# chaitjo/efficient-gnns

Measured on NVIDIA H100. Metric: edges aggregated/s (fwd+bwd), 3-layer GCN student + logit-KD, ARXIV-shape, higher is better.
Workload: dtype f32

## Files before the change

efficient-gnns_b200/csrc/gemm_wgrad_tf32x3.cu:

```cuda
#include "common.cuh"
#include "tc_common.cuh"

namespace b200gnn {
namespace wgrad {
using namespace tc;

constexpr int BKN = 32;
constexpr int TM = 128, TN = 128;
constexpr int THREADS = 384;
constexpr int STAGES = 5;
constexpr int X_BOX = 8;
constexpr int RAW_BYTES = BKN * (TM + TN) * 4;
constexpr int OP_BYTES = 128 * BKN * 4;
constexpr int T_BYTES = 2 * OP_BYTES;
constexpr int SS_BYTES = TM / 2 * 16;
constexpr int SMEM_BYTES = STAGES * RAW_BYTES + 2 * T_BYTES + 256 + SS_BYTES + 1024;
constexpr int MAX_RANGES = 132;
constexpr int64_t MAX_PARTIAL_FLOATS = (int64_t)MAX_RANGES * 256 * 256;
constexpr int MAX_KIN = 2048, MAX_NOUT = 512;
static_assert(SMEM_BYTES <= 232448, "shared memory");

struct Params {
  float* partial;
  int32_t Nn, Kin, Kpad, Nout, Npad, num_kb;
  int32_t n_tn, n_ranges;
  const float* act_scale;
  const float* act_shift;
  const uint32_t* act_bits;
  int32_t act_words;
  float inv_keep;
  const float* act_slope;
  int32_t act_ld;
};

template <bool ACT, bool PRELU = false>
__global__ void __launch_bounds__(THREADS, 1)
wgrad_tf32x3_kernel(const __grid_constant__ CUtensorMap tmX, const __grid_constant__ CUtensorMap tmG, const Params p) {
  extern __shared__ uint8_t smem_raw[];
  uint8_t* smem = reinterpret_cast<uint8_t*>((reinterpret_cast<uintptr_t>(smem_raw) + 1023) & ~(uintptr_t)1023);
  uint8_t* tbuf = smem + STAGES * RAW_BYTES;
  uint64_t* full = reinterpret_cast<uint64_t*>(tbuf + 2 * T_BYTES);
  uint64_t* empty = full + STAGES;
  float4* act_ss = reinterpret_cast<float4*>(tbuf + 2 * T_BYTES + 256);

  const int tiles = (p.Kpad / TM) * p.n_tn;
  const int tile = (int)blockIdx.x % tiles, range = (int)blockIdx.x / tiles;
  const int mt = tile / p.n_tn, nt = tile % p.n_tn;
  const int kb0 = (int)((int64_t)p.num_kb * range / p.n_ranges);
  const int kb1 = (int)((int64_t)p.num_kb * (range + 1) / p.n_ranges);

  const int warp = threadIdx.x >> 5, lane = threadIdx.x & 31;
  if (threadIdx.x == 0) {
    for (int s = 0; s < STAGES; ++s) { mbar_init(&full[s], 1); mbar_init(&empty[s], 256); }
    asm volatile("fence.mbarrier_init.release.cluster;" ::: "memory");
  }
  __syncthreads();

  if (warp < 4) {
    regs_dec<40>();
    if (threadIdx.x == 0) {
      int s = 0; uint32_t ph = 0;
      for (int kb = kb0; kb < kb1; ++kb) {
        mbar_wait(&empty[s], ph ^ 1);
        uint8_t* st = smem + s * RAW_BYTES;
        mbar_expect_tx(&full[s], RAW_BYTES);
        for (int j = 0; j < TM / X_BOX; ++j)
          tma_load_2d(&tmX, &full[s], st + j * BKN * X_BOX * 4, mt * TM + j * X_BOX, kb * BKN);
        tma_load_2d(&tmG, &full[s], st + BKN * TM * 4, nt * TN, kb * BKN);
        if (++s == STAGES) { s = 0; ph ^= 1; }
      }
    }
    return;
  }
  regs_inc<232>();

  const int cw = (warp >> 2) - 1;
  const int ct = threadIdx.x - 128;
  const uint32_t xfrag = (8 * cw + 2 * (warp & 3)) * (BKN * X_BOX * 4) + (lane & 3) * (X_BOX * 4) + (lane >> 2) * 4;
  const int pair = cw * 32 + (warp & 3) * 8 + (lane >> 2);
  const int c0 = mt * TM + cw * 64 + (warp & 3) * 16 + (lane >> 2);
  uint32_t wnext = 0u;
  const int bits_ld = PRELU ? p.act_ld : p.act_words;
  auto act_word = [&](int kb) {
    const int node = kb * BKN + lane;
    return node < p.Nn && (c0 >> 5) < p.act_words ? __ldg(p.act_bits + (size_t)node * bits_ld + (c0 >> 5)) : 0u;
  };
  const float slope = PRELU ? __ldg(p.act_slope) : 0.f;
  if (PRELU && kb0 < kb1) wnext = act_word(kb0);
  if (ACT) {
    if (ct < TM / 2) {
      const int c = mt * TM + (ct >> 3) * 16 + (ct & 7);
      float4 v = make_float4(0.f, 0.f, 0.f, 0.f);
      if (c < p.Kin) { v.x = __ldg(p.act_scale + c); v.y = __ldg(p.act_shift + c); }
      if (c + 8 < p.Kin) { v.z = __ldg(p.act_scale + c + 8); v.w = __ldg(p.act_shift + c + 8); }
      act_ss[ct] = v;
    }
    if (kb0 < kb1) wnext = act_word(kb0);
    named_sync(1, 256);
  }
  float acc[64], sum[64];
#pragma unroll
  for (int i = 0; i < 64; ++i) sum[i] = acc[i] = 0.f;
  uint32_t xh0[BKN / 8][4], xl0[BKN / 8][4], xh1[BKN / 8][4], xl1[BKN / 8][4];
  int s = 0; uint32_t ph = 0;
  auto block = [&](int i, uint32_t (&h)[BKN / 8][4], uint32_t (&l)[BKN / 8][4]) {
    uint32_t wcur = 0u;
    if (ACT || PRELU) {
      wcur = wnext;
      if (kb0 + i + 1 < kb1) wnext = act_word(kb0 + i + 1);
    }
    mbar_wait(&full[s], ph);
    float4 ss = make_float4(0.f, 0.f, 0.f, 0.f);
    int l4 = lane & 3;
    if (ACT) {
      ss = act_ss[pair];
      asm volatile("" : "+r"(l4));
    }
    if (PRELU) asm volatile("" : "+r"(l4));
    const uint32_t sraw = smem_u32(smem + s * RAW_BYTES);
    const float* rg = reinterpret_cast<const float*>(smem + s * RAW_BYTES + BKN * TM * 4);
    uint8_t* T = tbuf + (i & 1) * T_BYTES;
#pragma unroll
    for (int u = 0; u < 4; ++u) {
      const int idx = u * 256 + ct;
      const int r = idx & 127, c = idx >> 7;
      const float* src = rg + (4 * c) * 128 + r;
      const uint4 v = make_uint4(__float_as_uint(src[0]), __float_as_uint(src[128]), __float_as_uint(src[256]),
                                 __float_as_uint(src[384]));
      uint4 hv, lv;
      split4(v, hv, lv);
      *reinterpret_cast<uint4*>(T + swz128(r, c)) = hv;
      *reinterpret_cast<uint4*>(T + OP_BYTES + swz128(r, c)) = lv;
    }
#pragma unroll
    for (int k = 0; k < BKN / 8; ++k)
#pragma unroll
      for (int j = 0; j < 4; ++j) {
        uint32_t v = lds32(sraw + xfrag + (j & 1) * (BKN * X_BOX * 4) + (8 * k + 4 * (j >> 1)) * (X_BOX * 4));
        if (ACT) {
          const uint32_t w = __shfl_sync(0xffffffffu, wcur, 8 * k + l4 + 4 * (j >> 1));
          const float y = fmaxf(fmaf(__uint_as_float(v), (j & 1) ? ss.z : ss.x, (j & 1) ? ss.w : ss.y), 0.f) * p.inv_keep;
          v = (w >> ((c0 & 31) + 8 * (j & 1))) & 1u ? __float_as_uint(y) : 0u;
        }
        if (PRELU) {
          const uint32_t w = __shfl_sync(0xffffffffu, wcur, 8 * k + l4 + 4 * (j >> 1));
          const float z = __uint_as_float(v);
          const float y = (z > 0.f ? z : slope * z) * p.inv_keep;
          v = (w >> ((c0 & 31) + 8 * (j & 1))) & 1u ? __float_as_uint(y) : 0u;
        }
        split1(v, h[k][j], l[k][j]);
      }
    asm volatile("fence.proxy.async.shared::cta;" ::: "memory");
    mbar_arrive(&empty[s]);
    if (i > 0) {
      wgmma_wait<0>();
      acc_fence(acc);
#pragma unroll
      for (int j = 0; j < 64; ++j) sum[j] += acc[j];
    }
    named_sync(1, 256);
    reg_fence(h); reg_fence(l);
    wgmma_fence();
    const uint32_t sa = smem_u32(T);
#pragma unroll
    for (int k = 0; k < BKN / 8; ++k) {
      const uint32_t koff = k * 32;
      wgmma_tf32_n128_rs(acc, l[k], make_desc_k128(sa + koff), k != 0);
      wgmma_tf32_n128_rs(acc, h[k], make_desc_k128(sa + OP_BYTES + koff), 1);
    }
#pragma unroll
    for (int k = 0; k < BKN / 8; ++k) wgmma_tf32_n128_rs(acc, h[k], make_desc_k128(sa + k * 32), 1);
    wgmma_commit();
    if (++s == STAGES) { s = 0; ph ^= 1; }
  };
  for (int i = 0; i < kb1 - kb0; i += 2) {
    block(i, xh0, xl0);
    if (i + 1 < kb1 - kb0) block(i + 1, xh1, xl1);
  }
  if (kb1 > kb0) {
    wgmma_wait<0>();
    acc_fence(acc);
#pragma unroll
    for (int j = 0; j < 64; ++j) sum[j] += acc[j];
  }
  float* out = p.partial + (size_t)range * p.Kpad * p.Npad;
  const int row0 = mt * TM + cw * 64 + (warp & 3) * 16 + (lane >> 2);
#pragma unroll
  for (int j = 0; j < 16; ++j) {
    const int col = nt * TN + 8 * j + 2 * (lane & 3);
    if (col < p.Npad) {
      *reinterpret_cast<float2*>(out + (size_t)row0 * p.Npad + col) = make_float2(sum[4 * j], sum[4 * j + 1]);
      *reinterpret_cast<float2*>(out + (size_t)(row0 + 8) * p.Npad + col) = make_float2(sum[4 * j + 2], sum[4 * j + 3]);
    }
  }
}

constexpr int RED_VECS = 32, RED_GROUPS = 8;
__global__ void __launch_bounds__(RED_VECS * RED_GROUPS) wgrad_reduce_kernel(const float4* __restrict__ partial, int n_part,
                                                                             int Kin, int Kpad, int Nout, int Npad,
                                                                             float* __restrict__ out) {
  __shared__ float4 sh[RED_GROUPS][RED_VECS];
  const int64_t n_vec = (int64_t)Kpad * Npad / 4;
  const int v = threadIdx.x % RED_VECS, g = threadIdx.x / RED_VECS;
  const int64_t i = (int64_t)blockIdx.x * RED_VECS + v;
  float4 acc = make_float4(0.f, 0.f, 0.f, 0.f);
  if (i < n_vec)
    for (int c = g; c < n_part; c += RED_GROUPS) {
      const float4 x = __ldcs(partial + (size_t)c * n_vec + i);
      acc.x += x.x; acc.y += x.y; acc.z += x.z; acc.w += x.w;
    }
  sh[g][v] = acc;
  __syncthreads();
  if (g != 0 || i >= n_vec) return;
  const int row = (int)(i / (Npad / 4)), c4 = (int)(i % (Npad / 4)) * 4;
  if (c4 >= Nout || row >= Kin) return;
#pragma unroll
  for (int j = 1; j < RED_GROUPS; ++j) {
    const float4 x = sh[j][v];
    acc.x += x.x; acc.y += x.y; acc.z += x.z; acc.w += x.w;
  }
  *reinterpret_cast<float4*>(out + (size_t)row * Nout + c4) = acc;
}

static bool make_map_rows(CUtensorMap* m, const float* base, int64_t rows, int64_t width, int64_t ld, int box_cols) {
  EncodeTiledFn fn = encode_fn();
  if (!fn) return false;
  cuuint64_t dims[2] = {(cuuint64_t)width, (cuuint64_t)rows};
  cuuint64_t strides[1] = {(cuuint64_t)ld * 4};
  cuuint32_t box[2] = {(cuuint32_t)box_cols, (cuuint32_t)BKN};
  cuuint32_t estr[2] = {1, 1};
  return fn(m, CU_TENSOR_MAP_DATA_TYPE_FLOAT32, 2, const_cast<float*>(base), dims, strides, box, estr,
            CU_TENSOR_MAP_INTERLEAVE_NONE, CU_TENSOR_MAP_SWIZZLE_NONE, CU_TENSOR_MAP_L2_PROMOTION_L2_256B,
            CU_TENSOR_MAP_FLOAT_OOB_FILL_NONE) == CUDA_SUCCESS;
}

static int64_t pad_k(int64_t Kin) { return (Kin + TM - 1) / TM * TM; }
static int64_t pad_n(int64_t Nout) { return (Nout + 31) / 32 * 32; }
static int range_cap(int64_t Kin, int64_t Nout) {
  const int64_t c = MAX_PARTIAL_FLOATS / (pad_k(Kin) * pad_n(Nout));
  return (int)(c > MAX_RANGES ? MAX_RANGES : (c < 1 ? 1 : c));
}

}
}

using namespace b200gnn;

extern "C" int64_t b200gnn_wgrad_workspace_floats(int64_t Kin, int64_t Nout) {
  if (Kin <= 0 || Nout <= 0) return B200GNN_ERR_BAD_ARG;
  if (Kin > wgrad::MAX_KIN || Nout > wgrad::MAX_NOUT) return B200GNN_ERR_UNSUPPORTED;
  return wgrad::range_cap(Kin, Nout) * wgrad::pad_k(Kin) * wgrad::pad_n(Nout);
}

template <bool ACT, bool PRELU = false>
static int wgrad_launch(const float* X, int64_t ldx, const float* G, int64_t ldg, float* dW, int64_t Nn, int64_t Kin, int64_t Nout,
                        float* workspace, const wgrad::Params& act, void* stream) {
  if (!X || !G || !dW || !workspace || Nn <= 0 || Kin <= 0 || Nout <= 0 || ldx < Kin || ldg < Nout || Nn >= INT32_MAX)
    return B200GNN_ERR_BAD_ARG;
  if (Kin % 4 || Kin > wgrad::MAX_KIN || Nout % 4 || Nout > wgrad::MAX_NOUT || ldx % 4 || ldg % 4 || !aligned_to(X, 16) || !aligned_to(G, 16) ||
      !aligned_to(dW, 16) || !aligned_to(workspace, 16))
    return B200GNN_ERR_UNSUPPORTED;
  CUtensorMap tX, tG;
  if (!wgrad::make_map_rows(&tX, X, Nn, Kin, ldx, wgrad::X_BOX) || !wgrad::make_map_rows(&tG, G, Nn, Nout, ldg, wgrad::TN))
    return B200GNN_ERR_UNSUPPORTED;
  int dev = 0, sms = 132;
  cudaGetDevice(&dev);
  static bool attr_set[64] = {};
  if (dev >= 0 && dev < 64 && !attr_set[dev]) {
    cudaError_t e = cudaFuncSetAttribute(wgrad::wgrad_tf32x3_kernel<ACT, PRELU>, cudaFuncAttributeMaxDynamicSharedMemorySize,
                                         wgrad::SMEM_BYTES);
    if (e != cudaSuccess) { set_cuda_error(e); return B200GNN_ERR_CUDA; }
    attr_set[dev] = true;
  }
  cudaDeviceGetAttribute(&sms, cudaDevAttrMultiProcessorCount, dev);
  cudaStream_t st = (cudaStream_t)stream;
  wgrad::Params p = act;
  p.partial = workspace; p.Nn = (int32_t)Nn; p.Kin = (int32_t)Kin; p.Nout = (int32_t)Nout;
  p.Kpad = (int32_t)wgrad::pad_k(Kin);
  p.Npad = (int32_t)wgrad::pad_n(Nout);
  p.num_kb = (int32_t)((Nn + wgrad::BKN - 1) / wgrad::BKN);
  p.n_tn = (p.Npad + wgrad::TN - 1) / wgrad::TN;
  const int tiles = (int)(p.Kpad / wgrad::TM) * p.n_tn;
  int ranges = sms / tiles;
  const int cap = wgrad::range_cap(Kin, Nout);
  if (ranges > cap) ranges = cap;
  if (ranges > p.num_kb) ranges = p.num_kb;
  if (ranges < 1) ranges = 1;
  p.n_ranges = ranges;
  int rc;
  wgrad::wgrad_tf32x3_kernel<ACT, PRELU><<<tiles * ranges, wgrad::THREADS, wgrad::SMEM_BYTES, st>>>(tX, tG, p);
  if ((rc = check_launch())) return rc;
  const int64_t n_vec = (int64_t)p.Kpad * p.Npad / 4;
  wgrad::wgrad_reduce_kernel<<<(int)((n_vec + wgrad::RED_VECS - 1) / wgrad::RED_VECS), wgrad::RED_VECS * wgrad::RED_GROUPS, 0, st>>>(
      reinterpret_cast<const float4*>(workspace), ranges, (int)Kin, p.Kpad, (int)Nout, p.Npad, dW);
  return check_launch();
}

extern "C" int b200gnn_gemm_wgrad_tf32x3_f32(const float* X, int64_t ldx, const float* G, int64_t ldg, float* dW,
                                             int64_t Nn, int64_t Kin, int64_t Nout, float* workspace, void* stream) {
  return wgrad_launch<false>(X, ldx, G, ldg, dW, Nn, Kin, Nout, workspace, wgrad::Params{}, stream);
}

extern "C" int b200gnn_gemm_wgrad_tf32x3_act_f32(const float* Y, int64_t ldx, const float* G, int64_t ldg, float* dW,
                                                 int64_t Nn, int64_t Kin, int64_t Nout, const float* scale, const float* shift,
                                                 const uint32_t* bits, float p_drop, float* workspace, void* stream) {
  if (!scale || !shift || !bits || p_drop < 0.f || p_drop >= 1.f) return B200GNN_ERR_BAD_ARG;
  wgrad::Params act{};
  act.act_scale = scale; act.act_shift = shift; act.act_bits = bits; act.act_words = (int32_t)((Kin + 31) / 32);
  act.inv_keep = p_drop > 0.f ? 1.f / (1.f - p_drop) : 1.f;
  return wgrad_launch<true>(Y, ldx, G, ldg, dW, Nn, Kin, Nout, workspace, act, stream);
}

extern "C" int b200gnn_gemm_wgrad_tf32x3_prelu_f32(const float* Z, int64_t ldz, const float* G, int64_t ldg, float* dW,
                                                   int64_t Nn, int64_t Kin, int64_t Nout, const float* slope,
                                                   const uint32_t* bits, int64_t ldbits, float p_drop, float* workspace,
                                                   void* stream) {
  if (!slope || !bits || ldbits < (Kin + 31) / 32 || ldbits >= INT32_MAX || p_drop < 0.f || p_drop >= 1.f)
    return B200GNN_ERR_BAD_ARG;
  wgrad::Params act{};
  act.act_slope = slope; act.act_bits = bits; act.act_words = (int32_t)((Kin + 31) / 32); act.act_ld = (int32_t)ldbits;
  act.inv_keep = p_drop > 0.f ? 1.f / (1.f - p_drop) : 1.f;
  return wgrad_launch<false, true>(Z, ldz, G, ldg, dW, Nn, Kin, Nout, workspace, act, stream);
}
```

Baseline: 3.973 billion.

## Add narrow N=48 wgrad tile and offload half of transpose to producer warps

Templates the weight-gradient kernel on output tile width and dispatches a 48-wide tile (deeper pipeline, n48 wgmma) when Nout is small, as for the 40-class ArXiv output layer, instead of padding to 128. The G transpose/split work is also divided between the idle producer-side warps (96 threads) and the consumer warpgroups, coordinated by new tfull/tempty mbarriers that replace the named barrier. This cuts wasted MMA work on narrow outputs and overlaps the transpose with compute, at the cost of a more complex barrier protocol and some ablation macros left in the code.

```diff
diff --git a/efficient-gnns_b200/csrc/gemm_wgrad_tf32x3.cu b/efficient-gnns_b200/csrc/gemm_wgrad_tf32x3.cu
--- a/efficient-gnns_b200/csrc/gemm_wgrad_tf32x3.cu
+++ b/efficient-gnns_b200/csrc/gemm_wgrad_tf32x3.cu
@@ -1,24 +1,55 @@
 #include "common.cuh"
 #include "tc_common.cuh"
+
+#ifndef WGRAD_ABLATE
+#define WGRAD_ABLATE 0
+#endif
 
 namespace b200gnn {
 namespace wgrad {
 using namespace tc;
 
 constexpr int BKN = 32;
-constexpr int TM = 128, TN = 128;
+constexpr int TM = 128;
 constexpr int THREADS = 384;
-constexpr int STAGES = 5;
+constexpr int TRANSPOSERS = 96;
 constexpr int X_BOX = 8;
-constexpr int RAW_BYTES = BKN * (TM + TN) * 4;
-constexpr int OP_BYTES = 128 * BKN * 4;
-constexpr int T_BYTES = 2 * OP_BYTES;
 constexpr int SS_BYTES = TM / 2 * 16;
-constexpr int SMEM_BYTES = STAGES * RAW_BYTES + 2 * T_BYTES + 256 + SS_BYTES + 1024;
+constexpr int BAR_BYTES = 256;
+template <int TN>
+struct Tile {
+  static constexpr int STAGES = TN == 128 ? 5 : 8;
+  static constexpr int RAW_BYTES = BKN * (TM + TN) * 4;
+  static constexpr int OP_BYTES = TN * BKN * 4;
+  static constexpr int T_BYTES = 2 * OP_BYTES;
+  static constexpr int ACC = TN / 2;
+  static constexpr int SMEM_BYTES = STAGES * RAW_BYTES + 2 * T_BYTES + BAR_BYTES + SS_BYTES + 1024;
+  static_assert((STAGES * RAW_BYTES) % 1024 == 0 && OP_BYTES % 1024 == 0, "swizzled T tiles start on 1024-byte atoms");
+  static_assert((2 * STAGES + 4) * 8 <= BAR_BYTES, "barrier block");
+  static_assert(SMEM_BYTES <= 232448, "shared memory");
+};
 constexpr int MAX_RANGES = 132;
 constexpr int64_t MAX_PARTIAL_FLOATS = (int64_t)MAX_RANGES * 256 * 256;
 constexpr int MAX_KIN = 2048, MAX_NOUT = 512;
-static_assert(SMEM_BYTES <= 232448, "shared memory");
+
+__device__ __forceinline__ void mma(float (&d)[64], const uint32_t (&a)[4], uint64_t b, uint32_t s) { wgmma_tf32_n128_rs(d, a, b, s); }
+__device__ __forceinline__ void mma(float (&d)[24], const uint32_t (&a)[4], uint64_t b, uint32_t s) { wgmma_tf32_n48_rs(d, a, b, s); }
+
+template <int TN, int UNROLL>
+__device__ __forceinline__ void transpose_split(const float* rg, uint8_t* T, int idx, int end, int step) {
+  constexpr int OP_BYTES = TN * BKN * 4;
+#pragma unroll UNROLL
+  for (; idx < end; idx += step) {
+    const int r = idx % TN, c = idx / TN;
+    const float* src = rg + (4 * c) * TN + r;
+    const uint4 v = make_uint4(__float_as_uint(src[0]), __float_as_uint(src[TN]), __float_as_uint(src[2 * TN]),
+                               __float_as_uint(src[3 * TN]));
+    uint4 hv, lv;
+    split4(v, hv, lv);
+    *reinterpret_cast<uint4*>(T + swz128(r, c)) = hv;
+    *reinterpret_cast<uint4*>(T + OP_BYTES + swz128(r, c)) = lv;
+  }
+}
 
 struct Params {
   float* partial;
@@ -33,15 +64,19 @@
   int32_t act_ld;
 };
 
-template <bool ACT, bool PRELU = false>
+template <int TN, bool ACT, bool PRELU>
 __global__ void __launch_bounds__(THREADS, 1)
 wgrad_tf32x3_kernel(const __grid_constant__ CUtensorMap tmX, const __grid_constant__ CUtensorMap tmG, const Params p) {
+  using T_ = Tile<TN>;
+  constexpr int STAGES = T_::STAGES, RAW_BYTES = T_::RAW_BYTES, OP_BYTES = T_::OP_BYTES, T_BYTES = T_::T_BYTES;
   extern __shared__ uint8_t smem_raw[];
   uint8_t* smem = reinterpret_cast<uint8_t*>((reinterpret_cast<uintptr_t>(smem_raw) + 1023) & ~(uintptr_t)1023);
   uint8_t* tbuf = smem + STAGES * RAW_BYTES;
   uint64_t* full = reinterpret_cast<uint64_t*>(tbuf + 2 * T_BYTES);
   uint64_t* empty = full + STAGES;
-  float4* act_ss = reinterpret_cast<float4*>(tbuf + 2 * T_BYTES + 256);
+  uint64_t* tfull = empty + STAGES;
+  uint64_t* tempty = tfull + 2;
+  float4* act_ss = reinterpret_cast<float4*>(tbuf + 2 * T_BYTES + BAR_BYTES);
 
   const int tiles = (p.Kpad / TM) * p.n_tn;
   const int tile = (int)blockIdx.x % tiles, range = (int)blockIdx.x / tiles;
@@ -51,7 +86,8 @@
 
   const int warp = threadIdx.x >> 5, lane = threadIdx.x & 31;
   if (threadIdx.x == 0) {
-    for (int s = 0; s < STAGES; ++s) { mbar_init(&full[s], 1); mbar_init(&empty[s], 256); }
+    for (int s = 0; s < STAGES; ++s) { mbar_init(&full[s], 1); mbar_init(&empty[s], 256 + TRANSPOSERS); }
+    for (int t = 0; t < 2; ++t) { mbar_init(&tfull[t], TRANSPOSERS + 8); mbar_init(&tempty[t], 8); }
     asm volatile("fence.mbarrier_init.release.cluster;" ::: "memory");
   }
   __syncthreads();
@@ -67,6 +103,20 @@
         for (int j = 0; j < TM / X_BOX; ++j)
           tma_load_2d(&tmX, &full[s], st + j * BKN * X_BOX * 4, mt * TM + j * X_BOX, kb * BKN);
         tma_load_2d(&tmG, &full[s], st + BKN * TM * 4, nt * TN, kb * BKN);
+        if (++s == STAGES) { s = 0; ph ^= 1; }
+      }
+    } else if (warp > 0) {
+      const int tt = threadIdx.x - 32;
+      int s = 0; uint32_t ph = 0;
+      for (int i = 0; i < kb1 - kb0; ++i) {
+        const float* rg = reinterpret_cast<const float*>(smem + s * RAW_BYTES + BKN * TM * 4);
+        uint8_t* T = tbuf + (i & 1) * T_BYTES;
+        mbar_wait(&tempty[i & 1], ((i >> 1) & 1) ^ 1);
+        mbar_wait(&full[s], ph);
+        transpose_split<TN, 2>(rg, T, TN * BKN / 8 + tt, TN * BKN / 4 * (WGRAD_ABLATE != 2), TRANSPOSERS);
+        asm volatile("fence.proxy.async.shared::cta;" ::: "memory");
+        mbar_arrive(&empty[s]);
+        mbar_arrive(&tfull[i & 1]);
         if (++s == STAGES) { s = 0; ph ^= 1; }
       }
     }
@@ -98,9 +148,10 @@
     if (kb0 < kb1) wnext = act_word(kb0);
     named_sync(1, 256);
   }
-  float acc[64], sum[64];
-#pragma unroll
-  for (int i = 0; i < 64; ++i) sum[i] = acc[i] = 0.f;
+  constexpr int ACC = T_::ACC;
+  float acc[ACC], sum[ACC];
+#pragma unroll
+  for (int i = 0; i < ACC; ++i) sum[i] = acc[i] = 0.f;
   uint32_t xh0[BKN / 8][4], xl0[BKN / 8][4], xh1[BKN / 8][4], xl1[BKN / 8][4];
   int s = 0; uint32_t ph = 0;
   auto block = [&](int i, uint32_t (&h)[BKN / 8][4], uint32_t (&l)[BKN / 8][4]) {
@@ -117,21 +168,13 @@
       asm volatile("" : "+r"(l4));
     }
     if (PRELU) asm volatile("" : "+r"(l4));
+    mbar_wait(&tempty[i & 1], ((i >> 1) & 1) ^ 1);
+    transpose_split<TN, 1>(reinterpret_cast<const float*>(smem + s * RAW_BYTES + BKN * TM * 4), tbuf + (i & 1) * T_BYTES, ct,
+                        TN * BKN / 8 * (WGRAD_ABLATE != 2), 256);
+    asm volatile("fence.proxy.async.shared::cta;" ::: "memory");
+    __syncwarp();
+    if (lane == 0) mbar_arrive(&tfull[i & 1]);
     const uint32_t sraw = smem_u32(smem + s * RAW_BYTES);
-    const float* rg = reinterpret_cast<const float*>(smem + s * RAW_BYTES + BKN * TM * 4);
-    uint8_t* T = tbuf + (i & 1) * T_BYTES;
-#pragma unroll
-    for (int u = 0; u < 4; ++u) {
-      const int idx = u * 256 + ct;
-      const int r = idx & 127, c = idx >> 7;
-      const float* src = rg + (4 * c) * 128 + r;
-      const uint4 v = make_uint4(__float_as_uint(src[0]), __float_as_uint(src[128]), __float_as_uint(src[256]),
-                                 __float_as_uint(src[384]));
-      uint4 hv, lv;
-      split4(v, hv, lv);
-      *reinterpret_cast<uint4*>(T + swz128(r, c)) = hv;
-      *reinterpret_cast<uint4*>(T + OP_BYTES + swz128(r, c)) = lv;
-    }
 #pragma unroll
     for (int k = 0; k < BKN / 8; ++k)
 #pragma unroll
@@ -155,21 +198,22 @@
     if (i > 0) {
       wgmma_wait<0>();
       acc_fence(acc);
-#pragma unroll
-      for (int j = 0; j < 64; ++j) sum[j] += acc[j];
-    }
-    named_sync(1, 256);
+      if (lane == 0) mbar_arrive(&tempty[(i - 1) & 1]);
+#pragma unroll
+      for (int j = 0; j < ACC * (WGRAD_ABLATE != 3); ++j) sum[j] += acc[j];
+    }
+    mbar_wait(&tfull[i & 1], (i >> 1) & 1);
     reg_fence(h); reg_fence(l);
     wgmma_fence();
-    const uint32_t sa = smem_u32(T);
-#pragma unroll
-    for (int k = 0; k < BKN / 8; ++k) {
+    const uint32_t sa = smem_u32(tbuf + (i & 1) * T_BYTES);
+#pragma unroll
+    for (int k = 0; k < BKN / 8 * (WGRAD_ABLATE != 1); ++k) {
       const uint32_t koff = k * 32;
-      wgmma_tf32_n128_rs(acc, l[k], make_desc_k128(sa + koff), k != 0);
-      wgmma_tf32_n128_rs(acc, h[k], make_desc_k128(sa + OP_BYTES + koff), 1);
-    }
-#pragma unroll
-    for (int k = 0; k < BKN / 8; ++k) wgmma_tf32_n128_rs(acc, h[k], make_desc_k128(sa + k * 32), 1);
+      mma(acc, l[k], make_desc_k128(sa + koff), k != 0);
+      mma(acc, h[k], make_desc_k128(sa + OP_BYTES + koff), 1);
+    }
+#pragma unroll
+    for (int k = 0; k < BKN / 8 * (WGRAD_ABLATE != 1); ++k) mma(acc, h[k], make_desc_k128(sa + k * 32), 1);
     wgmma_commit();
     if (++s == STAGES) { s = 0; ph ^= 1; }
   };
@@ -181,12 +225,12 @@
     wgmma_wait<0>();
     acc_fence(acc);
 #pragma unroll
-    for (int j = 0; j < 64; ++j) sum[j] += acc[j];
+    for (int j = 0; j < ACC; ++j) sum[j] += acc[j];
   }
   float* out = p.partial + (size_t)range * p.Kpad * p.Npad;
   const int row0 = mt * TM + cw * 64 + (warp & 3) * 16 + (lane >> 2);
 #pragma unroll
-  for (int j = 0; j < 16; ++j) {
+  for (int j = 0; j < TN / 8; ++j) {
     const int col = nt * TN + 8 * j + 2 * (lane & 3);
     if (col < p.Npad) {
       *reinterpret_cast<float2*>(out + (size_t)row0 * p.Npad + col) = make_float2(sum[4 * j], sum[4 * j + 1]);
@@ -252,7 +296,7 @@
   return wgrad::range_cap(Kin, Nout) * wgrad::pad_k(Kin) * wgrad::pad_n(Nout);
 }
 
-template <bool ACT, bool PRELU = false>
+template <int TN, bool ACT, bool PRELU>
 static int wgrad_launch(const float* X, int64_t ldx, const float* G, int64_t ldg, float* dW, int64_t Nn, int64_t Kin, int64_t Nout,
                         float* workspace, const wgrad::Params& act, void* stream) {
   if (!X || !G || !dW || !workspace || Nn <= 0 || Kin <= 0 || Nout <= 0 || ldx < Kin || ldg < Nout || Nn >= INT32_MAX)
@@ -260,15 +304,16 @@
   if (Kin % 4 || Kin > wgrad::MAX_KIN || Nout % 4 || Nout > wgrad::MAX_NOUT || ldx % 4 || ldg % 4 || !aligned_to(X, 16) || !aligned_to(G, 16) ||
       !aligned_to(dW, 16) || !aligned_to(workspace, 16))
     return B200GNN_ERR_UNSUPPORTED;
+  constexpr int SMEM_BYTES = wgrad::Tile<TN>::SMEM_BYTES;
   CUtensorMap tX, tG;
-  if (!wgrad::make_map_rows(&tX, X, Nn, Kin, ldx, wgrad::X_BOX) || !wgrad::make_map_rows(&tG, G, Nn, Nout, ldg, wgrad::TN))
+  if (!wgrad::make_map_rows(&tX, X, Nn, Kin, ldx, wgrad::X_BOX) || !wgrad::make_map_rows(&tG, G, Nn, Nout, ldg, TN))
     return B200GNN_ERR_UNSUPPORTED;
   int dev = 0, sms = 132;
   cudaGetDevice(&dev);
   static bool attr_set[64] = {};
   if (dev >= 0 && dev < 64 && !attr_set[dev]) {
-    cudaError_t e = cudaFuncSetAttribute(wgrad::wgrad_tf32x3_kernel<ACT, PRELU>, cudaFuncAttributeMaxDynamicSharedMemorySize,
-                                         wgrad::SMEM_BYTES);
+    cudaError_t e = cudaFuncSetAttribute(wgrad::wgrad_tf32x3_kernel<TN, ACT, PRELU>, cudaFuncAttributeMaxDynamicSharedMemorySize,
+                                         SMEM_BYTES);
     if (e != cudaSuccess) { set_cuda_error(e); return B200GNN_ERR_CUDA; }
     attr_set[dev] = true;
   }
@@ -279,7 +324,7 @@
   p.Kpad = (int32_t)wgrad::pad_k(Kin);
   p.Npad = (int32_t)wgrad::pad_n(Nout);
   p.num_kb = (int32_t)((Nn + wgrad::BKN - 1) / wgrad::BKN);
-  p.n_tn = (p.Npad + wgrad::TN - 1) / wgrad::TN;
+  p.n_tn = (int32_t)((Nout + TN - 1) / TN);
   const int tiles = (int)(p.Kpad / wgrad::TM) * p.n_tn;
   int ranges = sms / tiles;
   const int cap = wgrad::range_cap(Kin, Nout);
@@ -288,7 +333,7 @@
   if (ranges < 1) ranges = 1;
   p.n_ranges = ranges;
   int rc;
-  wgrad::wgrad_tf32x3_kernel<ACT, PRELU><<<tiles * ranges, wgrad::THREADS, wgrad::SMEM_BYTES, st>>>(tX, tG, p);
+  wgrad::wgrad_tf32x3_kernel<TN, ACT, PRELU><<<tiles * ranges, wgrad::THREADS, SMEM_BYTES, st>>>(tX, tG, p);
   if ((rc = check_launch())) return rc;
   const int64_t n_vec = (int64_t)p.Kpad * p.Npad / 4;
   wgrad::wgrad_reduce_kernel<<<(int)((n_vec + wgrad::RED_VECS - 1) / wgrad::RED_VECS), wgrad::RED_VECS * wgrad::RED_GROUPS, 0, st>>>(
@@ -296,9 +341,16 @@
   return check_launch();
 }
 
+template <bool ACT, bool PRELU = false>
+static int wgrad_dispatch(const float* X, int64_t ldx, const float* G, int64_t ldg, float* dW, int64_t Nn, int64_t Kin,
+                          int64_t Nout, float* workspace, const wgrad::Params& act, void* stream) {
+  if (Nout <= 48) return wgrad_launch<48, ACT, PRELU>(X, ldx, G, ldg, dW, Nn, Kin, Nout, workspace, act, stream);
+  return wgrad_launch<128, ACT, PRELU>(X, ldx, G, ldg, dW, Nn, Kin, Nout, workspace, act, stream);
+}
+
 extern "C" int b200gnn_gemm_wgrad_tf32x3_f32(const float* X, int64_t ldx, const float* G, int64_t ldg, float* dW,
                                              int64_t Nn, int64_t Kin, int64_t Nout, float* workspace, void* stream) {
-  return wgrad_launch<false>(X, ldx, G, ldg, dW, Nn, Kin, Nout, workspace, wgrad::Params{}, stream);
+  return wgrad_dispatch<false>(X, ldx, G, ldg, dW, Nn, Kin, Nout, workspace, wgrad::Params{}, stream);
 }
 
 extern "C" int b200gnn_gemm_wgrad_tf32x3_act_f32(const float* Y, int64_t ldx, const float* G, int64_t ldg, float* dW,
@@ -308,7 +360,7 @@
   wgrad::Params act{};
   act.act_scale = scale; act.act_shift = shift; act.act_bits = bits; act.act_words = (int32_t)((Kin + 31) / 32);
   act.inv_keep = p_drop > 0.f ? 1.f / (1.f - p_drop) : 1.f;
-  return wgrad_launch<true>(Y, ldx, G, ldg, dW, Nn, Kin, Nout, workspace, act, stream);
+  return wgrad_dispatch<true>(Y, ldx, G, ldg, dW, Nn, Kin, Nout, workspace, act, stream);
 }
 
 extern "C" int b200gnn_gemm_wgrad_tf32x3_prelu_f32(const float* Z, int64_t ldz, const float* G, int64_t ldg, float* dW,
@@ -320,5 +372,5 @@
   wgrad::Params act{};
   act.act_slope = slope; act.act_bits = bits; act.act_words = (int32_t)((Kin + 31) / 32); act.act_ld = (int32_t)ldbits;
   act.inv_keep = p_drop > 0.f ? 1.f / (1.f - p_drop) : 1.f;
-  return wgrad_launch<false, true>(Z, ldz, G, ldg, dW, Nn, Kin, Nout, workspace, act, stream);
-}
+  return wgrad_dispatch<false, true>(Z, ldz, G, ldg, dW, Nn, Kin, Nout, workspace, act, stream);
+}
```

Result: faster. 4.064 billion (median of 6 runs) (+2.3%).
